# 610265158/Peppa_Pig_Face_Landmark

Hardware: NVIDIA H100
Metric: faces/sec Student@256 batch=256 (higher is better)
Workload: dtype f32

## Files before the change

### peppa_pig_face_landmark_b200/csrc/conv_fpw.cu

```cuda
#include <cuda.h>
#include <cuda_fp16.h>
#include <string.h>

#include "../../include/skps_b200.h"
#include "common.h"
#include "conv_fpw.h"
#include "tc_ptx.h"

namespace skps {

constexpr int FPW_PRODUCER_REGS = 32, FPW_TRANSFORM_REGS = 160, FPW_MMA_REGS = 160;
static_assert(128 * FPW_PRODUCER_REGS + 256 * FPW_TRANSFORM_REGS + 128 * FPW_MMA_REGS <= 65536, "register file split");

__device__ __forceinline__ float2 fpw_ld2(const void* base, int fmt, long long plane, long long i) {
    if (fmt == DT_SPLIT16) {
        const __half* h = (const __half*)base;
        const float2 a = __half22float2(*reinterpret_cast<const __half2*>(h + i));
        const float2 b = __half22float2(*reinterpret_cast<const __half2*>(h + i + plane));
        return make_float2(a.x + b.x, a.y + b.y);
    }
    return *reinterpret_cast<const float2*>((const float*)base + i);
}

template <int N, int KS>
__device__ __forceinline__ void fpw_mma(float* acc, uint64_t a_hi, uint64_t a_lo, uint64_t b_hi, uint64_t b_lo,
                                        uint32_t accumulate) {
    constexpr uint64_t A_HALF = 64 * 128 >> 4;
#pragma unroll
    for (int k = 0; k < KS; ++k) {
        const uint64_t koff = (uint64_t)(k * 32 >> 4);
#pragma unroll
        for (int m = 0; m < 2; ++m)
            wg_mma3<N>(acc + (N / 2) * m, a_hi + m * A_HALF + koff, a_lo + m * A_HALF + koff, b_hi + koff, b_lo + koff,
                       k ? 1u : accumulate);
    }
}

template <int MODE, int N, int ACT, bool OUT_SPLIT>
__global__ void __launch_bounds__(XF_THREADS, 1)
conv_fpw_kernel(const __grid_constant__ CUtensorMap tm0, const __grid_constant__ CUtensorMap tm1_hi,
                const __grid_constant__ CUtensorMap tm1_lo, const __grid_constant__ CUtensorMap tmB_hi,
                const __grid_constant__ CUtensorMap tmB_lo, const __grid_constant__ CUtensorMap tmO_hi,
                const __grid_constant__ CUtensorMap tmO_lo, const __grid_constant__ CUtensorMap tmW,
                const __grid_constant__ FpwK p) {
    extern __shared__ uint8_t smem_raw[];
    __shared__ __align__(8) XfBarriers bar;

    const int warp = threadIdx.x >> 5, lane = threadIdx.x & 31;
    const uint32_t b_plane = (uint32_t)N * 128u, b_slot = 2u * b_plane;
    const XfSmem sm = xf_smem<MODE>(smem_raw, p.a, p.bs, b_slot, p.out_bufs);
    xf_cta_init<MODE>(p.a, bar, sm, smem_raw, &tm0, &tm1_hi, &tmB_hi, &tmB_lo);
    if (warp < 4) {
        asm volatile("setmaxnreg.dec.sync.aligned.u32 %0;" ::"n"(FPW_PRODUCER_REGS));
    if (warp == 0) {
        if (lane == 0) {
            int st = 0, bst = 0;
            uint32_t ph = 0, bph = 0;
            for (int u = blockIdx.x; u < p.units; u += gridDim.x) {
                const int tile = u / p.nsplit, nh = u - tile * p.nsplit;
                const int img = tile / p.a.tiles_per_img, t = tile - img * p.a.tiles_per_img;
                const int oy0 = (t / p.a.tiles_x) * XF_TH, ox0 = (t % p.a.tiles_x) * XF_TW;
                for (int kc = 0; kc < p.a.cchunks; ++kc) {
                    mbar_wait_g(smem_u32(&bar.b_empty[bst]), bph ^ 1u);
                    const uint32_t fb = smem_u32(&bar.b_full[bst]);
                    mbar_expect_tx(fb, b_slot);
                    const uint32_t dst = sm.b_off + (uint32_t)bst * b_slot;
                    tma_load_2d(dst, &tmB_hi, fb, kc * 64, nh * N);
                    tma_load_2d(dst + b_plane, &tmB_lo, fb, kc * 64, nh * N);
                    if (++bst == p.bs) { bst = 0; bph ^= 1u; }
                    xf_load_a<MODE>(p.a, bar, sm, &tm0, &tm1_hi, &tm1_lo, &tmW, kc, img, oy0, ox0, st, ph);
                }
            }
        }
    }
    } else if (warp >= 8) {
        asm volatile("setmaxnreg.inc.sync.aligned.u32 %0;" ::"n"(FPW_TRANSFORM_REGS));
        xf_transform<MODE>(p.a, bar, sm, smem_raw, p.units, [&](int u) { return u / p.nsplit; });
    } else if (warp >= 4) {
        asm volatile("setmaxnreg.inc.sync.aligned.u32 %0;" ::"n"(FPW_MMA_REGS));
        const int q = warp & 3;
        const bool leader = q == 0 && lane == 0;
        int ast = 0, bst = 0;
        uint32_t aph = 0, bph = 0;
        int store_i = 0;
        for (int u = blockIdx.x; u < p.units; u += gridDim.x) {
            const int tile = u / p.nsplit, nh = u - tile * p.nsplit;
            float acc[N];
            int prev_a = 0, prev_b = 0;
            for (int kc = 0; kc < p.a.cchunks; ++kc) {
                mbar_wait_g(smem_u32(&bar.a_full[ast]), aph);
                mbar_wait_g(smem_u32(&bar.b_full[bst]), bph);
                const uint32_t sa = sm.a_off + (uint32_t)ast * XF_A_BYTES, sb = sm.b_off + (uint32_t)bst * b_slot;
                const uint64_t a_hi = make_smem_desc(sa), a_lo = make_smem_desc(sa + XF_A_PLANE);
                const uint64_t b_hi = make_smem_desc(sb), b_lo = make_smem_desc(sb + b_plane);
                const uint32_t accumulate = kc != 0;
                wg_fence_acc(acc);
                switch (p.a.chunk_ksteps[kc]) {
                    case 4: wg_fence(); fpw_mma<N, 4>(acc, a_hi, a_lo, b_hi, b_lo, accumulate); wg_commit(); break;
                    case 3: wg_fence(); fpw_mma<N, 3>(acc, a_hi, a_lo, b_hi, b_lo, accumulate); wg_commit(); break;
                    case 2: wg_fence(); fpw_mma<N, 2>(acc, a_hi, a_lo, b_hi, b_lo, accumulate); wg_commit(); break;
                    default: wg_fence(); fpw_mma<N, 1>(acc, a_hi, a_lo, b_hi, b_lo, accumulate); wg_commit(); break;
                }
                wg_fence_acc(acc);
                wg_wait<1>();
                wg_fence_acc(acc);
                if (kc > 0 && lane == 0) {
                    mbar_arrive(smem_u32(&bar.a_empty[prev_a]));
                    mbar_arrive(smem_u32(&bar.b_empty[prev_b]));
                }
                prev_a = ast; prev_b = bst;
                if (++ast == p.a.as) { ast = 0; aph ^= 1u; }
                if (++bst == p.bs) { bst = 0; bph ^= 1u; }
            }
            wg_wait<0>();
            wg_fence_acc(acc);
            if (lane == 0) {
                mbar_arrive(smem_u32(&bar.a_empty[prev_a]));
                mbar_arrive(smem_u32(&bar.b_empty[prev_b]));
            }
            const int img = tile / p.a.tiles_per_img, t = tile - img * p.a.tiles_per_img;
            const int ty0 = (t / p.a.tiles_x) * XF_TH, tx0 = (t % p.a.tiles_x) * XF_TW;
            const long long pix0 = ((long long)img * p.a.H + ty0) * p.a.W + tx0;
#pragma unroll
            for (int s = 0; s < (N + 31) / 32; ++s) {
                const int co = nh * N + 32 * s;
                if (co >= p.Cout) break;
                const uint32_t sbuf = sm.o_off + (uint32_t)(store_i % p.out_bufs) * XF_OUT_BUF;
                if (leader) {
                    if (p.out_bufs == 2) asm volatile("cp.async.bulk.wait_group.read 1;" ::: "memory");
                    else asm volatile("cp.async.bulk.wait_group.read 0;" ::: "memory");
                }
                ++store_i;
                asm volatile("bar.sync 1, 128;" ::: "memory");
                float bias[8];
#pragma unroll
                for (int i = 0; i < 4; ++i)
#pragma unroll
                    for (int j = 0; j < 2; ++j) {
                        const int c = co + 8 * i + 2 * (lane & 3) + j;
                        bias[2 * i + j] = c < p.Cout ? __ldg(p.bias + c) : 0.f;
                    }
#pragma unroll
                for (int m = 0; m < 2; ++m)
#pragma unroll
                    for (int h = 0; h < 2; ++h) {
                        const int r = 64 * m + 16 * q + (lane >> 2) + 8 * h;
#pragma unroll
                        for (int i = 0; i < 4; ++i) {
                            if (32 * s + 8 * i >= N) continue;
                            const float* a = acc + (N / 2) * m + 4 * (4 * s + i) + 2 * h;
                            float v0 = fmaf(a[0], p.out_scale, bias[2 * i]);
                            float v1 = fmaf(a[1], p.out_scale, bias[2 * i + 1]);
                            if (p.res && co + 8 * i < p.Cout) {
                                const long long pix = pix0 + (r / XF_TW) * p.a.W + r % XF_TW;
                                const float2 rv = fpw_ld2(p.res, p.res_fmt, p.res_plane,
                                                          pix * p.res_ld + p.res_coff + co + 8 * i + 2 * (lane & 3));
                                if (p.res_first) { v0 = act_t<ACT>(v0 + rv.x); v1 = act_t<ACT>(v1 + rv.y); }
                                else { v0 = act_t<ACT>(v0) + rv.x; v1 = act_t<ACT>(v1) + rv.y; }
                            } else {
                                v0 = act_t<ACT>(v0); v1 = act_t<ACT>(v1);
                            }
                            if (OUT_SPLIT) {
                                const __half2 h2 = __floats2half2_rn(v0, v1);
                                const float2 hf = __half22float2(h2);
                                const __half2 l2 = __floats2half2_rn(v0 - hf.x, v1 - hf.y);
                                const uint32_t addr = sbuf + (uint32_t)r * 64u + (uint32_t)((i ^ (r >> 1)) & 3) * 16u +
                                                      (uint32_t)(lane & 3) * 4u;
                                asm volatile("st.shared.b32 [%0], %1;" ::"r"(addr), "r"(*reinterpret_cast<const uint32_t*>(&h2)) : "memory");
                                asm volatile("st.shared.b32 [%0], %1;" ::"r"(addr + 8192u), "r"(*reinterpret_cast<const uint32_t*>(&l2)) : "memory");
                            } else {
                                const uint32_t addr = sbuf + (uint32_t)r * 128u +
                                                      (uint32_t)(((2 * i + ((lane & 3) >> 1)) ^ r) & 7) * 16u +
                                                      (uint32_t)(lane & 1) * 8u;
                                asm volatile("st.shared.v2.f32 [%0], {%1, %2};" ::"r"(addr), "f"(v0), "f"(v1) : "memory");
                            }
                        }
                    }
                asm volatile("fence.proxy.async.shared::cta;" ::: "memory");
                asm volatile("bar.sync 1, 128;" ::: "memory");
                if (leader) {
                    asm volatile("cp.async.bulk.tensor.4d.global.shared::cta.bulk_group [%0, {%2, %3, %4, %5}], [%1];"
                                 ::"l"(&tmO_hi), "r"(sbuf), "r"(co), "r"(tx0), "r"(ty0), "r"(img) : "memory");
                    if (OUT_SPLIT)
                        asm volatile("cp.async.bulk.tensor.4d.global.shared::cta.bulk_group [%0, {%2, %3, %4, %5}], [%1];"
                                     ::"l"(&tmO_lo), "r"(sbuf + 8192u), "r"(co), "r"(tx0), "r"(ty0), "r"(img) : "memory");
                    asm volatile("cp.async.bulk.commit_group;" ::: "memory");
                }
            }
        }
        if (leader) asm volatile("cp.async.bulk.wait_group 0;" ::: "memory");
    }
}

static int fpw_unit_width(int mode, int n_tile) {
    const int n = n_tile <= 64 ? n_tile : 64;
    if (mode == XF_DW) return n == 32 || n == 64 ? n : 0;
    return n == 48 || n == 64 ? n : 0;
}

bool fpw_supported(const XfSetup& s) {
    if (!xf_supported(s)) return false;
    if (s.act != ACT_NONE && s.act != ACT_RELU) return false;
    if (!fpw_unit_width(s.mode, s.n_tile)) return false;
    const TView& o = s.out;
    if (o.fmt != DT_SPLIT16 && o.fmt != DT_F32) return false;
    const size_t oes = o.fmt == DT_SPLIT16 ? 2 : 4;
    if (o.c_stride != 1 || (s.Cout % 8) || ((size_t)o.ld * oes) % 16 || ((size_t)o.c_off * oes) % 16) return false;
    if (((uintptr_t)o.base % 16) || (o.fmt == DT_SPLIT16 && ((size_t)o.plane * 2) % 16)) return false;
    if (o.H % XF_TH || o.W % XF_TW) return false;
    if (s.res.base) {
        if (s.res.c_stride != 1 || (s.res.fmt != DT_SPLIT16 && s.res.fmt != DT_F32)) return false;
        if (s.res.H != o.H || s.res.W != o.W || s.res.C < s.Cout || ((s.res.ld | s.res.c_off) & 1) || (s.res.plane & 1))
            return false;
    }
    XfProducer a;
    a.cchunks = ((s.low.base ? s.low.C : 0) + s.x.C + 63) / 64;
    int bs, out_bufs;
    return xf_rings(a, s.mode, (size_t)fpw_unit_width(s.mode, s.n_tile) * 256, 0, true, bs, out_bufs) != 0;
}

int fpw_prepare(FpwLayer& L, const XfSetup& s) {
    SKPS_CHECK(fpw_supported(s), "conv_fpw: unsupported layer");
    EncodeTiledFn enc = tensor_map_encoder();
    SKPS_CHECK(enc, "cuTensorMapEncodeTiled entry point not available");
    memset(&L.k, 0, sizeof(L.k));
    FpwK& k = L.k;
    L.mode = s.mode;
    L.n = fpw_unit_width(s.mode, s.n_tile);
    L.act = s.act;
    L.out_fmt = s.out.fmt;
    const TView& out = s.out;
    if (xf_producer_prepare(k.a, L.src0, L.src1_hi, L.src1_lo, L.w_eff, s)) return 1;
    k.nsplit = (s.n_tile + L.n - 1) / L.n;
    const int K_pad = k.a.cchunks * 64;
    for (int plane = 0; plane < 2; ++plane) {
        cuuint64_t dims[2] = {(cuuint64_t)K_pad, (cuuint64_t)s.n_tile};
        cuuint64_t strides[1] = {(cuuint64_t)K_pad * 2};
        cuuint32_t box[2] = {64, (cuuint32_t)L.n};
        cuuint32_t estr[2] = {1, 1};
        CUresult r = enc(plane ? &L.b_lo : &L.b_hi, CU_TENSOR_MAP_DATA_TYPE_FLOAT16, 2, (void*)(plane ? s.w_lo : s.w_hi), dims,
                         strides, box, estr, CU_TENSOR_MAP_INTERLEAVE_NONE, CU_TENSOR_MAP_SWIZZLE_128B,
                         CU_TENSOR_MAP_L2_PROMOTION_L2_256B, CU_TENSOR_MAP_FLOAT_OOB_FILL_NONE);
        SKPS_CHECK(r == CUDA_SUCCESS, "conv_fpw: cuTensorMapEncodeTiled(B) failed: %d", (int)r);
    }
    const bool split = out.fmt == DT_SPLIT16;
    const int oes = split ? 2 : 4;
    for (int plane = 0; plane < (split ? 2 : 1); ++plane) {
        cuuint64_t dims[4] = {(cuuint64_t)s.Cout, (cuuint64_t)out.W, (cuuint64_t)out.H, (cuuint64_t)s.max_batch};
        cuuint64_t strides[3] = {(cuuint64_t)out.ld * oes, (cuuint64_t)out.W * out.ld * oes,
                                 (cuuint64_t)out.H * out.W * out.ld * oes};
        cuuint32_t box[4] = {32, XF_TW, XF_TH, 1};
        cuuint32_t estr[4] = {1, 1, 1, 1};
        char* base = (char*)out.base + (size_t)out.c_off * oes + (plane ? (size_t)out.plane * 2 : 0);
        CUresult r = enc(plane ? &L.o_lo : &L.o_hi, split ? CU_TENSOR_MAP_DATA_TYPE_FLOAT16 : CU_TENSOR_MAP_DATA_TYPE_FLOAT32,
                         4, base, dims, strides, box, estr, CU_TENSOR_MAP_INTERLEAVE_NONE,
                         split ? CU_TENSOR_MAP_SWIZZLE_64B : CU_TENSOR_MAP_SWIZZLE_128B, CU_TENSOR_MAP_L2_PROMOTION_NONE,
                         CU_TENSOR_MAP_FLOAT_OOB_FILL_NONE);
        SKPS_CHECK(r == CUDA_SUCCESS, "conv_fpw: cuTensorMapEncodeTiled(out) failed: %d", (int)r);
    }
    if (!split) L.o_lo = L.o_hi;
    const size_t smem = xf_rings(k.a, s.mode, (size_t)L.n * 256, 0, true, k.bs, k.out_bufs);
    SKPS_CHECK(smem, "conv_fpw: layer does not fit shared memory");
    L.smem_bytes = (int)smem + 1024;
    k.Cout = s.Cout; k.out_scale = s.out_scale;
    k.bias = s.bias ? s.bias : zero_bias();
    SKPS_CHECK(k.bias, "conv_fpw: zero-bias allocation failed");
    k.res = s.res.base; k.res_fmt = s.res.fmt; k.res_plane = s.res.plane; k.res_ld = s.res.ld; k.res_coff = s.res.c_off;
    k.res_first = s.res.base ? s.res_first : 0;
    return 0;
}

template <int MODE, int N, int ACT, bool SPLIT>
static int fpw_launch_t(const FpwLayer& L, const FpwK& k, int grid, cudaStream_t stream) {
    static int attr_bytes[MAX_DEVICES] = {};
    if (smem_limit((const void*)conv_fpw_kernel<MODE, N, ACT, SPLIT>, attr_bytes, L.smem_bytes)) return 1;
    conv_fpw_kernel<MODE, N, ACT, SPLIT><<<grid, XF_THREADS, L.smem_bytes, stream>>>(
        L.src0, L.src1_hi, L.src1_lo, L.b_hi, L.b_lo, L.o_hi, L.o_lo, L.w_eff, k);
    SKPS_CUDA(cudaGetLastError());
    return 0;
}

template <int MODE, int N>
static int fpw_launch_n(const FpwLayer& L, const FpwK& k, int grid, cudaStream_t stream) {
    const bool sp = L.out_fmt == DT_SPLIT16;
    switch (L.act) {
        case ACT_NONE: return sp ? fpw_launch_t<MODE, N, ACT_NONE, true>(L, k, grid, stream) : fpw_launch_t<MODE, N, ACT_NONE, false>(L, k, grid, stream);
        case ACT_RELU: return sp ? fpw_launch_t<MODE, N, ACT_RELU, true>(L, k, grid, stream) : fpw_launch_t<MODE, N, ACT_RELU, false>(L, k, grid, stream);
        default: break;
    }
    set_error("conv_fpw: activation %d not instantiated", L.act);
    return 1;
}

Grid fpw_grid(const FpwLayer& L, int batch, int num_sms, FpwK* kp) {
    FpwK k = L.k;
    k.units = batch * k.a.tiles_per_img * k.nsplit;
    if (kp) *kp = k;
    return persistent_grid(k.units, num_sms);
}

int fpw_launch(const FpwLayer& L, int batch, int num_sms, cudaStream_t stream) {
    FpwK k;
    const int grid = fpw_grid(L, batch, num_sms, &k).ctas;
    if (L.mode == XF_DW) {
        switch (L.n) {
            case 32: return fpw_launch_n<XF_DW, 32>(L, k, grid, stream);
            case 64: return fpw_launch_n<XF_DW, 64>(L, k, grid, stream);
            default: break;
        }
    } else {
        switch (L.n) {
            case 48: return fpw_launch_n<XF_SCALE, 48>(L, k, grid, stream);
            case 64: return fpw_launch_n<XF_SCALE, 64>(L, k, grid, stream);
            default: break;
        }
    }
    set_error("conv_fpw: mode %d width %d not instantiated", L.mode, L.n);
    return 1;
}

}
```

### peppa_pig_face_landmark_b200/csrc/conv_fpw.h

```cpp
#pragma once
#include <cuda.h>
#include <cuda_runtime.h>
#include <stdint.h>

#include "xf_producer.h"

namespace skps {

struct FpwK {
    XfProducer a;
    int units;
    int nsplit;
    int bs, out_bufs;
    int Cout;
    float out_scale;
    const float* bias;
    const void* res; int res_fmt; long long res_plane; int res_ld, res_coff; int res_first;
};

struct FpwLayer {
    CUtensorMap src0, src1_hi, src1_lo, b_hi, b_lo, o_hi, o_lo, w_eff;
    FpwK k;
    int mode = 0, n = 0, act = 0, out_fmt = 0;
    int smem_bytes = 0;
};

bool fpw_supported(const XfSetup& s);
int fpw_prepare(FpwLayer& L, const XfSetup& s);
Grid fpw_grid(const FpwLayer& L, int batch, int num_sms, FpwK* k = nullptr);
int fpw_launch(const FpwLayer& L, int batch, int num_sms, cudaStream_t stream);

}
```

### peppa_pig_face_landmark_b200/csrc/xf_producer.h

```cpp
#pragma once
#include <cuda.h>
#include <cuda_fp16.h>
#include <cuda_runtime.h>
#include <stdint.h>

#include "common.h"
#include "tc_ptx.h"

namespace skps {

enum { XF_SCALE = 0, XF_DW = 1 };
enum { XS_UP_F32 = 0, XS_DW_F32 = 1, XS_DW_SPLIT = 2 };
constexpr int XF_MAX_CHUNKS = 16;

constexpr int XF_THREADS = 512;
constexpr int XF_TW = 16, XF_TH = 8;
constexpr int XF_IW = XF_TW + 2, XF_IH = XF_TH + 2;
constexpr int XF_LW = XF_TW / 2 + 2, XF_LH = XF_TH / 2 + 2;
constexpr int XF_RAW_BYTES = XF_IH * XF_IW * 128;
constexpr int XF_UP_BYTES = XF_LH * XF_LW * 128;
constexpr int XF_A_PLANE = 128 * 128;
constexpr int XF_A_BYTES = 2 * XF_A_PLANE;
constexpr int XF_RING = 4;
constexpr int XF_OUT_BUF = 16384;

struct XfSetup {
    int mode;
    int max_batch;
    TView x, low, gate;
    const float* dww;
    const float* weff;
    int dw_act;
    int Cout, act, n_tile, n_tiles;
    float out_scale;
    const void* w_hi; const void* w_lo;
    const float* bias;
    TView out, res;
    int res_first;
};

struct XfProducer {
    int H, W, tiles_x, tiles_per_img;
    int cchunks, Cin;
    int rs, as;
    int dw_act;
    int Hl, Wl;
    int halves;
    int wcx;
    uint8_t sub_mode[2 * XF_MAX_CHUNKS];
    int16_t sub_c[2 * XF_MAX_CHUNKS];
    uint8_t chunk_subs[XF_MAX_CHUNKS];
    uint8_t chunk_ksteps[XF_MAX_CHUNKS];
    const float* dww;
    const float* gate; int gate_ld, gate_coff;
};

bool xf_supported(const XfSetup& s);
int xf_producer_prepare(XfProducer& k, CUtensorMap& src0, CUtensorMap& src1_hi, CUtensorMap& src1_lo, CUtensorMap& w_eff,
                        const XfSetup& s);
size_t xf_rings(XfProducer& k, int mode, size_t b_slot, size_t reserve, bool two_out_bufs, int& bs, int& out_bufs);

struct XfBarriers {
    uint64_t raw_full[XF_RING], raw_empty[XF_RING], a_raw[XF_RING], a_full[XF_RING], a_empty[XF_RING], b_full[XF_RING],
        b_empty[XF_RING];
};

struct XfSmem {
    uint32_t a_off, b_off, o_off, r_off, w_off;
};

template <int MODE>
__device__ __forceinline__ XfSmem xf_smem(const uint8_t* smem_raw, const XfProducer& p, int bs, uint32_t b_slot, int out_bufs) {
    XfSmem s;
    s.a_off = (smem_u32(smem_raw) + 1023u) & ~1023u;
    s.b_off = s.a_off + (uint32_t)p.as * XF_A_BYTES;
    s.o_off = s.b_off + (uint32_t)bs * b_slot;
    s.r_off = s.o_off + (uint32_t)out_bufs * XF_OUT_BUF;
    s.w_off = s.r_off + (MODE == XF_DW ? (uint32_t)p.rs * XF_RAW_BYTES : 0u);
    return s;
}

template <int MODE>
__device__ __forceinline__ void xf_cta_init(const XfProducer& p, XfBarriers& bar, const XfSmem& sm, uint8_t* smem_raw,
                                            const CUtensorMap* tm0, const CUtensorMap* tm1_hi, const CUtensorMap* tmB_hi,
                                            const CUtensorMap* tmB_lo) {
    const int warp = threadIdx.x >> 5, lane = threadIdx.x & 31;
    if (warp == 0 && lane == 0) {
        asm volatile("prefetch.tensormap [%0];" ::"l"(tm0) : "memory");
        asm volatile("prefetch.tensormap [%0];" ::"l"(tm1_hi) : "memory");
        asm volatile("prefetch.tensormap [%0];" ::"l"(tmB_hi) : "memory");
        asm volatile("prefetch.tensormap [%0];" ::"l"(tmB_lo) : "memory");
    }
    if (warp == 1 && lane == 0) {
        for (int s = 0; s < XF_RING; ++s) {
            mbar_init(smem_u32(&bar.raw_full[s]), 1);
            mbar_init(smem_u32(&bar.raw_empty[s]), p.halves ? 4 : 8);
            mbar_init(smem_u32(&bar.a_raw[s]), 1);
            mbar_init(smem_u32(&bar.a_full[s]), 8);
            mbar_init(smem_u32(&bar.a_empty[s]), 4);
            mbar_init(smem_u32(&bar.b_full[s]), 1);
            mbar_init(smem_u32(&bar.b_empty[s]), 4);
        }
        asm volatile("fence.mbarrier_init.release.cluster;" ::: "memory");
    }
    if (MODE == XF_DW) {
        float* dws = reinterpret_cast<float*>(smem_raw + (sm.w_off - smem_u32(smem_raw)));
        for (int i = threadIdx.x; i < 10 * p.cchunks * 64; i += XF_THREADS) dws[i] = __ldg(p.dww + i);
    }
    __syncthreads();
}

template <int MODE>
__device__ __forceinline__ void xf_load_a(const XfProducer& p, XfBarriers& bar, const XfSmem& sm, const CUtensorMap* tm0,
                                          const CUtensorMap* tm1_hi, const CUtensorMap* tm1_lo, const CUtensorMap* tmW,
                                          int kc, int img, int oy0, int ox0, int& st, uint32_t& ph) {
    if (MODE == XF_SCALE) {
        mbar_wait_g(smem_u32(&bar.a_empty[st]), ph ^ 1u);
        const uint32_t fb = smem_u32(&bar.a_raw[st]);
        mbar_expect_tx(fb, XF_A_BYTES);
        const uint32_t dst = sm.a_off + (uint32_t)st * XF_A_BYTES;
        tma_load_4d(dst, tm1_hi, fb, kc * 64, ox0, oy0, img);
        tma_load_4d(dst + XF_A_PLANE, tm1_lo, fb, kc * 64, ox0, oy0, img);
        if (++st == p.as) { st = 0; ph ^= 1u; }
        return;
    }
    const int subs = p.chunk_subs[kc];
    for (int h = 0; h < subs; ++h) {
        const int si = kc * 2 + h, smode = p.sub_mode[si], c = p.sub_c[si];
        mbar_wait_g(smem_u32(&bar.raw_empty[st]), ph ^ 1u);
        const uint32_t fb = smem_u32(&bar.raw_full[st]);
        const uint32_t dst = sm.r_off + (uint32_t)st * XF_RAW_BYTES;
        if (smode == XS_UP_F32) {
            mbar_expect_tx(fb, XF_UP_BYTES + (uint32_t)p.wcx * 3u * 9u * 128u);
            tma_load_4d(dst, tm0, fb, c, (ox0 >> 1) - 1, (oy0 >> 1) - 1, img);
            tma_load_5d(dst + XF_UP_BYTES, tmW, fb, 0, 0, (p.wcx == 4 || ox0 == 0) ? 0 : 1, oy0 == 0 ? 0 : 1, c >> 5);
        } else if (smode == XS_DW_F32) {
            mbar_expect_tx(fb, XF_RAW_BYTES);
            tma_load_4d(dst, tm0, fb, c, ox0 - 1, oy0 - 1, img);
        } else {
            mbar_expect_tx(fb, XF_RAW_BYTES);
            tma_load_4d(dst, tm1_hi, fb, c, ox0 - 1, oy0 - 1, img);
            tma_load_4d(dst + XF_RAW_BYTES / 2, tm1_lo, fb, c, ox0 - 1, oy0 - 1, img);
        }
        if (++st == p.rs) { st = 0; ph ^= 1u; }
    }
}

__device__ __forceinline__ void split_store4(uint32_t addr_hi, const float4 v) {
    const __half2 h01 = __floats2half2_rn(v.x, v.y), h23 = __floats2half2_rn(v.z, v.w);
    const float2 f01 = __half22float2(h01), f23 = __half22float2(h23);
    const __half2 l01 = __floats2half2_rn(v.x - f01.x, v.y - f01.y), l23 = __floats2half2_rn(v.z - f23.x, v.w - f23.y);
    asm volatile("st.shared.v2.b32 [%0], {%1, %2};" ::"r"(addr_hi), "r"(*reinterpret_cast<const uint32_t*>(&h01)),
                 "r"(*reinterpret_cast<const uint32_t*>(&h23)) : "memory");
    asm volatile("st.shared.v2.b32 [%0], {%1, %2};" ::"r"(addr_hi + (uint32_t)XF_A_PLANE),
                 "r"(*reinterpret_cast<const uint32_t*>(&l01)), "r"(*reinterpret_cast<const uint32_t*>(&l23)) : "memory");
}
__device__ __forceinline__ float4 f4_fma(const float4 a, const float4 w, const float4 c) {
    return make_float4(fmaf(a.x, w.x, c.x), fmaf(a.y, w.y, c.y), fmaf(a.z, w.z, c.z), fmaf(a.w, w.w, c.w));
}

template <int ACT>
__device__ __forceinline__ void act16(float4* acc) {
#pragma unroll
    for (int q = 0; q < 4; ++q) {
        acc[q].x = act_t<ACT>(acc[q].x); acc[q].y = act_t<ACT>(acc[q].y);
        acc[q].z = act_t<ACT>(acc[q].z); acc[q].w = act_t<ACT>(acc[q].w);
    }
}

template <int MODE, class TileOf>
__device__ __forceinline__ void xf_transform(const XfProducer& p, XfBarriers& bar, const XfSmem& sm, uint8_t* smem_raw,
                                             int n_work, TileOf tile_of) {
    const int lane = threadIdx.x & 31;
    const int tt = threadIdx.x - 256;
    const int Kpad = p.cchunks * 64;
    int ast = 0, rst = 0;
    uint32_t aph = 0, rph = 0;
    if (MODE == XF_SCALE) {
        const int r0 = tt >> 3, ps = tt & 7, j = ps ^ (r0 & 7);
        for (int u = blockIdx.x; u < n_work; u += gridDim.x) {
            const int img = tile_of(u) / p.tiles_per_img;
            const float* grow = p.gate + (long long)img * p.gate_ld + p.gate_coff;
            for (int kc = 0; kc < p.cchunks; ++kc) {
                const int c = kc * 64 + j * 8;
                float g[8];
                if (c < p.Cin) {
                    const float4 g0 = __ldg(reinterpret_cast<const float4*>(grow + c));
                    const float4 g1 = __ldg(reinterpret_cast<const float4*>(grow + c + 4));
                    g[0] = g0.x; g[1] = g0.y; g[2] = g0.z; g[3] = g0.w; g[4] = g1.x; g[5] = g1.y; g[6] = g1.z; g[7] = g1.w;
                } else {
#pragma unroll
                    for (int e = 0; e < 8; ++e) g[e] = 0.f;
                }
                mbar_wait_g(smem_u32(&bar.a_raw[ast]), aph);
                const uint32_t sa = sm.a_off + (uint32_t)ast * XF_A_BYTES + (uint32_t)ps * 16u;
#pragma unroll
                for (int i = 0; i < 4; ++i) {
                    const uint32_t ad = sa + (uint32_t)(r0 + 32 * i) * 128u;
                    uint32_t hv[4], lv[4];
                    asm volatile("ld.shared.v4.b32 {%0, %1, %2, %3}, [%4];" : "=r"(hv[0]), "=r"(hv[1]), "=r"(hv[2]), "=r"(hv[3]) : "r"(ad) : "memory");
                    asm volatile("ld.shared.v4.b32 {%0, %1, %2, %3}, [%4];" : "=r"(lv[0]), "=r"(lv[1]), "=r"(lv[2]), "=r"(lv[3]) : "r"(ad + (uint32_t)XF_A_PLANE) : "memory");
#pragma unroll
                    for (int e = 0; e < 4; ++e) {
                        const float2 hf = __half22float2(*reinterpret_cast<const __half2*>(&hv[e]));
                        const float2 lf = __half22float2(*reinterpret_cast<const __half2*>(&lv[e]));
                        const float v0 = (hf.x + lf.x) * g[2 * e], v1 = (hf.y + lf.y) * g[2 * e + 1];
                        const __half2 h2 = __floats2half2_rn(v0, v1);
                        const float2 h2f = __half22float2(h2);
                        const __half2 l2 = __floats2half2_rn(v0 - h2f.x, v1 - h2f.y);
                        hv[e] = *reinterpret_cast<const uint32_t*>(&h2);
                        lv[e] = *reinterpret_cast<const uint32_t*>(&l2);
                    }
                    asm volatile("st.shared.v4.b32 [%0], {%1, %2, %3, %4};" ::"r"(ad), "r"(hv[0]), "r"(hv[1]), "r"(hv[2]), "r"(hv[3]) : "memory");
                    asm volatile("st.shared.v4.b32 [%0], {%1, %2, %3, %4};" ::"r"(ad + (uint32_t)XF_A_PLANE), "r"(lv[0]), "r"(lv[1]), "r"(lv[2]), "r"(lv[3]) : "memory");
                }
                asm volatile("fence.proxy.async.shared::cta;" ::: "memory");
                __syncwarp();
                if (lane == 0) mbar_arrive(smem_u32(&bar.a_full[ast]));
                if (++ast == p.as) { ast = 0; aph ^= 1u; }
            }
        }
    } else if (!p.halves) {
        const int cl = tt & 7, pg = tt >> 3, prow = pg >> 2, xs = (pg & 3) * 4;
        const float* dws = reinterpret_cast<const float*>(smem_raw + (sm.w_off - smem_u32(smem_raw)));
        for (int u = blockIdx.x; u < n_work; u += gridDim.x) {
            for (int kc = 0; kc < p.cchunks; ++kc) {
                mbar_wait_g(smem_u32(&bar.a_empty[ast]), aph ^ 1u);
                const uint32_t sa = sm.a_off + (uint32_t)ast * XF_A_BYTES;
                const int subs = p.chunk_subs[kc];
                for (int h = 0; h < subs; ++h) {
                    const int smode = p.sub_mode[kc * 2 + h];
                    const int cw = kc * 64 + h * 32 + cl * 4;
                    const float4 bias4 = *reinterpret_cast<const float4*>(dws + 9 * Kpad + cw);
                    float4 acc[4] = {bias4, bias4, bias4, bias4};
                    mbar_wait_g(smem_u32(&bar.raw_full[rst]), rph);
                    const uint8_t* raw = smem_raw + (sm.r_off + (uint32_t)rst * XF_RAW_BYTES - smem_u32(smem_raw));
                    {
#pragma unroll
                        for (int ky = 0; ky < 3; ++ky) {
                            float4 in[6];
#pragma unroll
                            for (int i = 0; i < 6; ++i) {
                                const int px = (prow + ky) * XF_IW + xs + i;
                                if (smode == XS_DW_F32) {
                                    in[i] = *reinterpret_cast<const float4*>(raw + (px * 32 + cl * 4) * 4);
                                } else {
                                    const uint2 a = *reinterpret_cast<const uint2*>(raw + (px * 32 + cl * 4) * 2);
                                    const uint2 b = *reinterpret_cast<const uint2*>(raw + XF_RAW_BYTES / 2 + (px * 32 + cl * 4) * 2);
                                    const float2 a01 = __half22float2(*reinterpret_cast<const __half2*>(&a.x));
                                    const float2 a23 = __half22float2(*reinterpret_cast<const __half2*>(&a.y));
                                    const float2 b01 = __half22float2(*reinterpret_cast<const __half2*>(&b.x));
                                    const float2 b23 = __half22float2(*reinterpret_cast<const __half2*>(&b.y));
                                    in[i] = make_float4(a01.x + b01.x, a01.y + b01.y, a23.x + b23.x, a23.y + b23.y);
                                }
                            }
#pragma unroll
                            for (int kx = 0; kx < 3; ++kx) {
                                const float4 w = *reinterpret_cast<const float4*>(dws + (ky * 3 + kx) * Kpad + cw);
#pragma unroll
                                for (int q = 0; q < 4; ++q) acc[q] = f4_fma(in[q + kx], w, acc[q]);
// ... 170 lines not shown
```

Measured before the change: 20180.

## Add paired-consumer fused pointwise kernel sharing one A tile across two N halves

After: 20800 (median of 6 runs). 1.03x the previous value.

```diff
diff --git a/peppa_pig_face_landmark_b200/csrc/conv_fpw.cu b/peppa_pig_face_landmark_b200/csrc/conv_fpw.cu
--- a/peppa_pig_face_landmark_b200/csrc/conv_fpw.cu
+++ b/peppa_pig_face_landmark_b200/csrc/conv_fpw.cu
@@ -33,6 +33,152 @@
         for (int m = 0; m < 2; ++m)
             wg_mma3<N>(acc + (N / 2) * m, a_hi + m * A_HALF + koff, a_lo + m * A_HALF + koff, b_hi + koff, b_lo + koff,
                        k ? 1u : accumulate);
+    }
+}
+
+template <int N, int ACT, bool OUT_SPLIT, int PER, bool RES>
+__device__ __forceinline__ void fpw_consumer(const FpwK& p, XfBarriers& bar, const XfSmem& sm, const CUtensorMap* tmO_hi,
+                                             const CUtensorMap* tmO_lo, int wg) {
+    const int warp = threadIdx.x >> 5, lane = threadIdx.x & 31;
+    const uint32_t b_plane = (uint32_t)(PER * N) * 128u, b_slot = 2u * b_plane, b_row = (uint32_t)(wg * N) * 128u;
+    const uint32_t o_base = sm.o_off + (uint32_t)(wg * p.out_bufs) * XF_OUT_BUF, named_bar = 1 + wg;
+    const int items = p.nsplit / PER;
+    const int q = warp & 3;
+    const bool leader = q == 0 && lane == 0;
+    int ast = 0, bst = 0;
+    uint32_t aph = 0, bph = 0;
+    int store_i = 0;
+    for (int u = blockIdx.x; u < p.units; u += gridDim.x) {
+        const int tile = u / items, nh = (u - tile * items) * PER + wg;
+        float acc[N];
+        int prev_a = 0, prev_b = 0;
+        for (int kc = 0; kc < p.a.cchunks; ++kc) {
+            mbar_wait_g(smem_u32(&bar.a_full[ast]), aph);
+            mbar_wait_g(smem_u32(&bar.b_full[bst]), bph);
+            const uint32_t sa = sm.a_off + (uint32_t)ast * XF_A_BYTES, sb = sm.b_off + (uint32_t)bst * b_slot + b_row;
+            const uint64_t a_hi = make_smem_desc(sa), a_lo = make_smem_desc(sa + XF_A_PLANE);
+            const uint64_t b_hi = make_smem_desc(sb), b_lo = make_smem_desc(sb + b_plane);
+            const uint32_t accumulate = kc != 0;
+            wg_fence_acc(acc);
+            switch (p.a.chunk_ksteps[kc]) {
+                case 4: wg_fence(); fpw_mma<N, 4>(acc, a_hi, a_lo, b_hi, b_lo, accumulate); wg_commit(); break;
+                case 3: wg_fence(); fpw_mma<N, 3>(acc, a_hi, a_lo, b_hi, b_lo, accumulate); wg_commit(); break;
+                case 2: wg_fence(); fpw_mma<N, 2>(acc, a_hi, a_lo, b_hi, b_lo, accumulate); wg_commit(); break;
+                default: wg_fence(); fpw_mma<N, 1>(acc, a_hi, a_lo, b_hi, b_lo, accumulate); wg_commit(); break;
+            }
+            wg_fence_acc(acc);
+            wg_wait<1>();
+            wg_fence_acc(acc);
+            if (kc > 0 && lane == 0) {
+                mbar_arrive(smem_u32(&bar.a_empty[prev_a]));
+                mbar_arrive(smem_u32(&bar.b_empty[prev_b]));
+            }
+            prev_a = ast; prev_b = bst;
+            if (++ast == p.a.as) { ast = 0; aph ^= 1u; }
+            if (++bst == p.bs) { bst = 0; bph ^= 1u; }
+        }
+        wg_wait<0>();
+        wg_fence_acc(acc);
+        if (lane == 0) {
+            mbar_arrive(smem_u32(&bar.a_empty[prev_a]));
+            mbar_arrive(smem_u32(&bar.b_empty[prev_b]));
+        }
+        const int img = tile / p.a.tiles_per_img, t = tile - img * p.a.tiles_per_img;
+        const int ty0 = (t / p.a.tiles_x) * XF_TH, tx0 = (t % p.a.tiles_x) * XF_TW;
+        const long long pix0 = ((long long)img * p.a.H + ty0) * p.a.W + tx0;
+#pragma unroll
+        for (int s = 0; s < (N + 31) / 32; ++s) {
+            const int co = nh * N + 32 * s;
+            if (co >= p.Cout) break;
+            const uint32_t sbuf = o_base + (uint32_t)(store_i % p.out_bufs) * XF_OUT_BUF;
+            if (leader) {
+                if (p.out_bufs == 2) asm volatile("cp.async.bulk.wait_group.read 1;" ::: "memory");
+                else asm volatile("cp.async.bulk.wait_group.read 0;" ::: "memory");
+            }
+            ++store_i;
+            asm volatile("bar.sync %0, 128;" ::"r"(named_bar) : "memory");
+            float bias[8];
+#pragma unroll
+            for (int i = 0; i < 4; ++i)
+#pragma unroll
+                for (int j = 0; j < 2; ++j) {
+                    const int c = co + 8 * i + 2 * (lane & 3) + j;
+                    bias[2 * i + j] = c < p.Cout ? __ldg(p.bias + c) : 0.f;
+                }
+#pragma unroll
+            for (int m = 0; m < 2; ++m)
+#pragma unroll
+                for (int h = 0; h < 2; ++h) {
+                    const int r = 64 * m + 16 * q + (lane >> 2) + 8 * h;
+#pragma unroll
+                    for (int i = 0; i < 4; ++i) {
+                        if (32 * s + 8 * i >= N) continue;
+                        const float* a = acc + (N / 2) * m + 4 * (4 * s + i) + 2 * h;
+                        float v0 = fmaf(a[0], p.out_scale, bias[2 * i]);
+                        float v1 = fmaf(a[1], p.out_scale, bias[2 * i + 1]);
+                        if (RES && p.res && co + 8 * i < p.Cout) {
+                            const long long pix = pix0 + (r / XF_TW) * p.a.W + r % XF_TW;
+                            const float2 rv = fpw_ld2(p.res, p.res_fmt, p.res_plane,
+                                                      pix * p.res_ld + p.res_coff + co + 8 * i + 2 * (lane & 3));
+                            if (p.res_first) { v0 = act_t<ACT>(v0 + rv.x); v1 = act_t<ACT>(v1 + rv.y); }
+                            else { v0 = act_t<ACT>(v0) + rv.x; v1 = act_t<ACT>(v1) + rv.y; }
+                        } else {
+                            v0 = act_t<ACT>(v0); v1 = act_t<ACT>(v1);
+                        }
+                        if (OUT_SPLIT) {
+                            const __half2 h2 = __floats2half2_rn(v0, v1);
+                            const float2 hf = __half22float2(h2);
+                            const __half2 l2 = __floats2half2_rn(v0 - hf.x, v1 - hf.y);
+                            const uint32_t addr = sbuf + (uint32_t)r * 64u + (uint32_t)((i ^ (r >> 1)) & 3) * 16u +
+                                                  (uint32_t)(lane & 3) * 4u;
+                            asm volatile("st.shared.b32 [%0], %1;" ::"r"(addr), "r"(*reinterpret_cast<const uint32_t*>(&h2)) : "memory");
+                            asm volatile("st.shared.b32 [%0], %1;" ::"r"(addr + 8192u), "r"(*reinterpret_cast<const uint32_t*>(&l2)) : "memory");
+                        } else {
+                            const uint32_t addr = sbuf + (uint32_t)r * 128u +
+                                                  (uint32_t)(((2 * i + ((lane & 3) >> 1)) ^ r) & 7) * 16u +
+                                                  (uint32_t)(lane & 1) * 8u;
+                            asm volatile("st.shared.v2.f32 [%0], {%1, %2};" ::"r"(addr), "f"(v0), "f"(v1) : "memory");
+                        }
+                    }
+                }
+            asm volatile("fence.proxy.async.shared::cta;" ::: "memory");
+            asm volatile("bar.sync %0, 128;" ::"r"(named_bar) : "memory");
+            if (leader) {
+                asm volatile("cp.async.bulk.tensor.4d.global.shared::cta.bulk_group [%0, {%2, %3, %4, %5}], [%1];"
+                             ::"l"(tmO_hi), "r"(sbuf), "r"(co), "r"(tx0), "r"(ty0), "r"(img) : "memory");
+                if (OUT_SPLIT)
+                    asm volatile("cp.async.bulk.tensor.4d.global.shared::cta.bulk_group [%0, {%2, %3, %4, %5}], [%1];"
+                                 ::"l"(tmO_lo), "r"(sbuf + 8192u), "r"(co), "r"(tx0), "r"(ty0), "r"(img) : "memory");
+                asm volatile("cp.async.bulk.commit_group;" ::: "memory");
+            }
+        }
+    }
+    if (leader) asm volatile("cp.async.bulk.wait_group 0;" ::: "memory");
+}
+
+template <int MODE, int N, int PER>
+__device__ __forceinline__ void fpw_producer(const FpwK& p, XfBarriers& bar, const XfSmem& sm, const CUtensorMap* tm0,
+                                             const CUtensorMap* tm1_hi, const CUtensorMap* tm1_lo,
+                                             const CUtensorMap* tmB_hi, const CUtensorMap* tmB_lo,
+                                             const CUtensorMap* tmW) {
+    const uint32_t b_plane = (uint32_t)(PER * N) * 128u, b_slot = 2u * b_plane;
+    const int items = p.nsplit / PER;
+    int st = 0, bst = 0;
+    uint32_t ph = 0, bph = 0;
+    for (int u = blockIdx.x; u < p.units; u += gridDim.x) {
+        const int tile = u / items, n0 = (u - tile * items) * PER * N;
+        const int img = tile / p.a.tiles_per_img, t = tile - img * p.a.tiles_per_img;
+        const int oy0 = (t / p.a.tiles_x) * XF_TH, ox0 = (t % p.a.tiles_x) * XF_TW;
+        for (int kc = 0; kc < p.a.cchunks; ++kc) {
+            mbar_wait_g(smem_u32(&bar.b_empty[bst]), bph ^ 1u);
+            const uint32_t fb = smem_u32(&bar.b_full[bst]);
+            mbar_expect_tx(fb, b_slot);
+            const uint32_t dst = sm.b_off + (uint32_t)bst * b_slot;
+            tma_load_2d(dst, tmB_hi, fb, kc * 64, n0);
+            tma_load_2d(dst + b_plane, tmB_lo, fb, kc * 64, n0);
+            if (++bst == p.bs) { bst = 0; bph ^= 1u; }
+            xf_load_a<MODE>(p.a, bar, sm, tm0, tm1_hi, tm1_lo, tmW, kc, img, oy0, ox0, st, ph);
+        }
     }
 }
 
@@ -47,148 +193,48 @@
     __shared__ __align__(8) XfBarriers bar;
 
     const int warp = threadIdx.x >> 5, lane = threadIdx.x & 31;
-    const uint32_t b_plane = (uint32_t)N * 128u, b_slot = 2u * b_plane;
-    const XfSmem sm = xf_smem<MODE>(smem_raw, p.a, p.bs, b_slot, p.out_bufs);
+    const XfSmem sm = xf_smem<MODE>(smem_raw, p.a, p.bs, 2u * N * 128u, p.out_bufs);
     xf_cta_init<MODE>(p.a, bar, sm, smem_raw, &tm0, &tm1_hi, &tmB_hi, &tmB_lo);
     if (warp < 4) {
         asm volatile("setmaxnreg.dec.sync.aligned.u32 %0;" ::"n"(FPW_PRODUCER_REGS));
-    if (warp == 0) {
-        if (lane == 0) {
-            int st = 0, bst = 0;
-            uint32_t ph = 0, bph = 0;
-            for (int u = blockIdx.x; u < p.units; u += gridDim.x) {
-                const int tile = u / p.nsplit, nh = u - tile * p.nsplit;
-                const int img = tile / p.a.tiles_per_img, t = tile - img * p.a.tiles_per_img;
-                const int oy0 = (t / p.a.tiles_x) * XF_TH, ox0 = (t % p.a.tiles_x) * XF_TW;
-                for (int kc = 0; kc < p.a.cchunks; ++kc) {
-                    mbar_wait_g(smem_u32(&bar.b_empty[bst]), bph ^ 1u);
-                    const uint32_t fb = smem_u32(&bar.b_full[bst]);
-                    mbar_expect_tx(fb, b_slot);
-                    const uint32_t dst = sm.b_off + (uint32_t)bst * b_slot;
-                    tma_load_2d(dst, &tmB_hi, fb, kc * 64, nh * N);
-                    tma_load_2d(dst + b_plane, &tmB_lo, fb, kc * 64, nh * N);
-                    if (++bst == p.bs) { bst = 0; bph ^= 1u; }
-                    xf_load_a<MODE>(p.a, bar, sm, &tm0, &tm1_hi, &tm1_lo, &tmW, kc, img, oy0, ox0, st, ph);
-                }
-            }
-        }
-    }
+        if (warp == 0 && lane == 0) fpw_producer<MODE, N, 1>(p, bar, sm, &tm0, &tm1_hi, &tm1_lo, &tmB_hi, &tmB_lo, &tmW);
     } else if (warp >= 8) {
         asm volatile("setmaxnreg.inc.sync.aligned.u32 %0;" ::"n"(FPW_TRANSFORM_REGS));
         xf_transform<MODE>(p.a, bar, sm, smem_raw, p.units, [&](int u) { return u / p.nsplit; });
-    } else if (warp >= 4) {
+    } else {
         asm volatile("setmaxnreg.inc.sync.aligned.u32 %0;" ::"n"(FPW_MMA_REGS));
-        const int q = warp & 3;
-        const bool leader = q == 0 && lane == 0;
-        int ast = 0, bst = 0;
-        uint32_t aph = 0, bph = 0;
-        int store_i = 0;
-        for (int u = blockIdx.x; u < p.units; u += gridDim.x) {
-            const int tile = u / p.nsplit, nh = u - tile * p.nsplit;
-            float acc[N];
-            int prev_a = 0, prev_b = 0;
-            for (int kc = 0; kc < p.a.cchunks; ++kc) {
-                mbar_wait_g(smem_u32(&bar.a_full[ast]), aph);
-                mbar_wait_g(smem_u32(&bar.b_full[bst]), bph);
-                const uint32_t sa = sm.a_off + (uint32_t)ast * XF_A_BYTES, sb = sm.b_off + (uint32_t)bst * b_slot;
-                const uint64_t a_hi = make_smem_desc(sa), a_lo = make_smem_desc(sa + XF_A_PLANE);
-                const uint64_t b_hi = make_smem_desc(sb), b_lo = make_smem_desc(sb + b_plane);
-                const uint32_t accumulate = kc != 0;
-                wg_fence_acc(acc);
-                switch (p.a.chunk_ksteps[kc]) {
-                    case 4: wg_fence(); fpw_mma<N, 4>(acc, a_hi, a_lo, b_hi, b_lo, accumulate); wg_commit(); break;
-                    case 3: wg_fence(); fpw_mma<N, 3>(acc, a_hi, a_lo, b_hi, b_lo, accumulate); wg_commit(); break;
-                    case 2: wg_fence(); fpw_mma<N, 2>(acc, a_hi, a_lo, b_hi, b_lo, accumulate); wg_commit(); break;
-                    default: wg_fence(); fpw_mma<N, 1>(acc, a_hi, a_lo, b_hi, b_lo, accumulate); wg_commit(); break;
-                }
-                wg_fence_acc(acc);
-                wg_wait<1>();
-                wg_fence_acc(acc);
-                if (kc > 0 && lane == 0) {
-                    mbar_arrive(smem_u32(&bar.a_empty[prev_a]));
-                    mbar_arrive(smem_u32(&bar.b_empty[prev_b]));
-                }
-                prev_a = ast; prev_b = bst;
-                if (++ast == p.a.as) { ast = 0; aph ^= 1u; }
-                if (++bst == p.bs) { bst = 0; bph ^= 1u; }
-            }
-            wg_wait<0>();
-            wg_fence_acc(acc);
-            if (lane == 0) {
-                mbar_arrive(smem_u32(&bar.a_empty[prev_a]));
-                mbar_arrive(smem_u32(&bar.b_empty[prev_b]));
-            }
-            const int img = tile / p.a.tiles_per_img, t = tile - img * p.a.tiles_per_img;
-            const int ty0 = (t / p.a.tiles_x) * XF_TH, tx0 = (t % p.a.tiles_x) * XF_TW;
-            const long long pix0 = ((long long)img * p.a.H + ty0) * p.a.W + tx0;
-#pragma unroll
-            for (int s = 0; s < (N + 31) / 32; ++s) {
-                const int co = nh * N + 32 * s;
-                if (co >= p.Cout) break;
-                const uint32_t sbuf = sm.o_off + (uint32_t)(store_i % p.out_bufs) * XF_OUT_BUF;
-                if (leader) {
-                    if (p.out_bufs == 2) asm volatile("cp.async.bulk.wait_group.read 1;" ::: "memory");
-                    else asm volatile("cp.async.bulk.wait_group.read 0;" ::: "memory");
-                }
-                ++store_i;
-                asm volatile("bar.sync 1, 128;" ::: "memory");
-                float bias[8];
-#pragma unroll
-                for (int i = 0; i < 4; ++i)
-#pragma unroll
-                    for (int j = 0; j < 2; ++j) {
-                        const int c = co + 8 * i + 2 * (lane & 3) + j;
-                        bias[2 * i + j] = c < p.Cout ? __ldg(p.bias + c) : 0.f;
-                    }
-#pragma unroll
-                for (int m = 0; m < 2; ++m)
-#pragma unroll
-                    for (int h = 0; h < 2; ++h) {
-                        const int r = 64 * m + 16 * q + (lane >> 2) + 8 * h;
-#pragma unroll
-                        for (int i = 0; i < 4; ++i) {
-                            if (32 * s + 8 * i >= N) continue;
-                            const float* a = acc + (N / 2) * m + 4 * (4 * s + i) + 2 * h;
-                            float v0 = fmaf(a[0], p.out_scale, bias[2 * i]);
-                            float v1 = fmaf(a[1], p.out_scale, bias[2 * i + 1]);
-                            if (p.res && co + 8 * i < p.Cout) {
-                                const long long pix = pix0 + (r / XF_TW) * p.a.W + r % XF_TW;
-                                const float2 rv = fpw_ld2(p.res, p.res_fmt, p.res_plane,
-                                                          pix * p.res_ld + p.res_coff + co + 8 * i + 2 * (lane & 3));
-                                if (p.res_first) { v0 = act_t<ACT>(v0 + rv.x); v1 = act_t<ACT>(v1 + rv.y); }
-                                else { v0 = act_t<ACT>(v0) + rv.x; v1 = act_t<ACT>(v1) + rv.y; }
-                            } else {
-                                v0 = act_t<ACT>(v0); v1 = act_t<ACT>(v1);
-                            }
-                            if (OUT_SPLIT) {
-                                const __half2 h2 = __floats2half2_rn(v0, v1);
-                                const float2 hf = __half22float2(h2);
-                                const __half2 l2 = __floats2half2_rn(v0 - hf.x, v1 - hf.y);
-                                const uint32_t addr = sbuf + (uint32_t)r * 64u + (uint32_t)((i ^ (r >> 1)) & 3) * 16u +
-                                                      (uint32_t)(lane & 3) * 4u;
-                                asm volatile("st.shared.b32 [%0], %1;" ::"r"(addr), "r"(*reinterpret_cast<const uint32_t*>(&h2)) : "memory");
-                                asm volatile("st.shared.b32 [%0], %1;" ::"r"(addr + 8192u), "r"(*reinterpret_cast<const uint32_t*>(&l2)) : "memory");
-                            } else {
-                                const uint32_t addr = sbuf + (uint32_t)r * 128u +
-                                                      (uint32_t)(((2 * i + ((lane & 3) >> 1)) ^ r) & 7) * 16u +
-                                                      (uint32_t)(lane & 1) * 8u;
-                                asm volatile("st.shared.v2.f32 [%0], {%1, %2};" ::"r"(addr), "f"(v0), "f"(v1) : "memory");
-                            }
-                        }
-                    }
-                asm volatile("fence.proxy.async.shared::cta;" ::: "memory");
-                asm volatile("bar.sync 1, 128;" ::: "memory");
-                if (leader) {
-                    asm volatile("cp.async.bulk.tensor.4d.global.shared::cta.bulk_group [%0, {%2, %3, %4, %5}], [%1];"
-                                 ::"l"(&tmO_hi), "r"(sbuf), "r"(co), "r"(tx0), "r"(ty0), "r"(img) : "memory");
-                    if (OUT_SPLIT)
-                        asm volatile("cp.async.bulk.tensor.4d.global.shared::cta.bulk_group [%0, {%2, %3, %4, %5}], [%1];"
-                                     ::"l"(&tmO_lo), "r"(sbuf + 8192u), "r"(co), "r"(tx0), "r"(ty0), "r"(img) : "memory");
-                    asm volatile("cp.async.bulk.commit_group;" ::: "memory");
-                }
-            }
-        }
-        if (leader) asm volatile("cp.async.bulk.wait_group 0;" ::: "memory");
+        fpw_consumer<N, ACT, OUT_SPLIT, 1, true>(p, bar, sm, &tmO_hi, &tmO_lo, 0);
+    }
+}
+
+constexpr int FPW_PAIR_THREADS = 640;
+constexpr int FPW_PAIR_PRODUCER_REGS = 24, FPW_PAIR_TRANSFORM_REGS = 120, FPW_PAIR_MMA_REGS = 104;
+static_assert(128 * FPW_PAIR_PRODUCER_REGS + 256 * FPW_PAIR_TRANSFORM_REGS + 256 * FPW_PAIR_MMA_REGS <= FPW_PAIR_THREADS * 96,
+              "register file split");
+
+template <int ACT, bool OUT_SPLIT>
+__global__ void __launch_bounds__(FPW_PAIR_THREADS, 1)
+conv_fpw_pair(const __grid_constant__ CUtensorMap tm0, const __grid_constant__ CUtensorMap tm1_hi,
+              const __grid_constant__ CUtensorMap tm1_lo, const __grid_constant__ CUtensorMap tmB_hi,
+              const __grid_constant__ CUtensorMap tmB_lo, const __grid_constant__ CUtensorMap tmO_hi,
+              const __grid_constant__ CUtensorMap tmO_lo, const __grid_constant__ CUtensorMap tmW,
+              const __grid_constant__ FpwK p) {
+    constexpr int N = 64;
+    extern __shared__ uint8_t smem_raw[];
+    __shared__ __align__(8) XfBarriers bar;
+
+    const int warp = threadIdx.x >> 5, lane = threadIdx.x & 31;
+    const XfSmem sm = xf_smem<XF_DW>(smem_raw, p.a, p.bs, 4u * N * 128u, 2 * p.out_bufs);
+    xf_cta_init<XF_DW>(p.a, bar, sm, smem_raw, &tm0, &tm1_hi, &tmB_hi, &tmB_lo, 8, FPW_PAIR_THREADS);
+    if (warp < 4) {
+        asm volatile("setmaxnreg.dec.sync.aligned.u32 %0;" ::"n"(FPW_PAIR_PRODUCER_REGS));
+        if (warp == 0 && lane == 0) fpw_producer<XF_DW, N, 2>(p, bar, sm, &tm0, &tm1_hi, &tm1_lo, &tmB_hi, &tmB_lo, &tmW);
+    } else if (warp >= 8 && warp < 16) {
+        asm volatile("setmaxnreg.inc.sync.aligned.u32 %0;" ::"n"(FPW_PAIR_TRANSFORM_REGS));
+        xf_transform<XF_DW>(p.a, bar, sm, smem_raw, p.units, [&](int u) { return u / (p.nsplit / 2); });
+    } else {
+        asm volatile("setmaxnreg.inc.sync.aligned.u32 %0;" ::"n"(FPW_PAIR_MMA_REGS));
+        fpw_consumer<N, ACT, OUT_SPLIT, 2, false>(p, bar, sm, &tmO_hi, &tmO_lo, warp < 8 ? 0 : 1);
     }
 }
 
@@ -196,6 +242,17 @@
     const int n = n_tile <= 64 ? n_tile : 64;
     if (mode == XF_DW) return n == 32 || n == 64 ? n : 0;
     return n == 48 || n == 64 ? n : 0;
+}
+
+static bool fpw_pair(const XfSetup& s) {
+    const int n = fpw_unit_width(s.mode, s.n_tile);
+    return s.mode == XF_DW && n == 64 && (s.n_tile + n - 1) / n % 2 == 0 && !s.res.base;
+}
+
+static size_t fpw_rings(XfProducer& a, const XfSetup& s, int& bs, int& out_bufs) {
+    const size_t n = (size_t)fpw_unit_width(s.mode, s.n_tile);
+    if (fpw_pair(s)) return xf_rings(a, s.mode, 2 * n * 256, XF_OUT_BUF, false, bs, out_bufs) + XF_OUT_BUF;
+    return xf_rings(a, s.mode, n * 256, 0, true, bs, out_bufs);
 }
 
 bool fpw_supported(const XfSetup& s) {
@@ -216,7 +273,7 @@
     XfProducer a;
     a.cchunks = ((s.low.base ? s.low.C : 0) + s.x.C + 63) / 64;
     int bs, out_bufs;
-    return xf_rings(a, s.mode, (size_t)fpw_unit_width(s.mode, s.n_tile) * 256, 0, true, bs, out_bufs) != 0;
+    return fpw_rings(a, s, bs, out_bufs) != 0;
 }
 
 int fpw_prepare(FpwLayer& L, const XfSetup& s) {
@@ -227,6 +284,7 @@
     FpwK& k = L.k;
     L.mode = s.mode;
     L.n = fpw_unit_width(s.mode, s.n_tile);
+    L.pair = fpw_pair(s);
     L.act = s.act;
     L.out_fmt = s.out.fmt;
     const TView& out = s.out;
@@ -236,7 +294,7 @@
     for (int plane = 0; plane < 2; ++plane) {
         cuuint64_t dims[2] = {(cuuint64_t)K_pad, (cuuint64_t)s.n_tile};
         cuuint64_t strides[1] = {(cuuint64_t)K_pad * 2};
-        cuuint32_t box[2] = {64, (cuuint32_t)L.n};
+        cuuint32_t box[2] = {64, (cuuint32_t)(L.pair ? 2 * L.n : L.n)};
         cuuint32_t estr[2] = {1, 1};
         CUresult r = enc(plane ? &L.b_lo : &L.b_hi, CU_TENSOR_MAP_DATA_TYPE_FLOAT16, 2, (void*)(plane ? s.w_lo : s.w_hi), dims,
                          strides, box, estr, CU_TENSOR_MAP_INTERLEAVE_NONE, CU_TENSOR_MAP_SWIZZLE_128B,
@@ -259,7 +317,7 @@
         SKPS_CHECK(r == CUDA_SUCCESS, "conv_fpw: cuTensorMapEncodeTiled(out) failed: %d", (int)r);
     }
     if (!split) L.o_lo = L.o_hi;
-    const size_t smem = xf_rings(k.a, s.mode, (size_t)L.n * 256, 0, true, k.bs, k.out_bufs);
+    const size_t smem = fpw_rings(k.a, s, k.bs, k.out_bufs);
     SKPS_CHECK(smem, "conv_fpw: layer does not fit shared memory");
     L.smem_bytes = (int)smem + 1024;
     k.Cout = s.Cout; k.out_scale = s.out_scale;
@@ -280,6 +338,27 @@
     return 0;
 }
 
+template <int ACT, bool SPLIT>
+static int fpw_launch_pair_t(const FpwLayer& L, const FpwK& k, int grid, cudaStream_t stream) {
+    static int attr_bytes[MAX_DEVICES] = {};
+    if (smem_limit((const void*)conv_fpw_pair<ACT, SPLIT>, attr_bytes, L.smem_bytes)) return 1;
+    conv_fpw_pair<ACT, SPLIT><<<grid, FPW_PAIR_THREADS, L.smem_bytes, stream>>>(
+        L.src0, L.src1_hi, L.src1_lo, L.b_hi, L.b_lo, L.o_hi, L.o_lo, L.w_eff, k);
+    SKPS_CUDA(cudaGetLastError());
+    return 0;
+}
+
+static int fpw_launch_pair(const FpwLayer& L, const FpwK& k, int grid, cudaStream_t stream) {
+    const bool sp = L.out_fmt == DT_SPLIT16;
+    switch (L.act) {
+        case ACT_NONE: return sp ? fpw_launch_pair_t<ACT_NONE, true>(L, k, grid, stream) : fpw_launch_pair_t<ACT_NONE, false>(L, k, grid, stream);
+        case ACT_RELU: return sp ? fpw_launch_pair_t<ACT_RELU, true>(L, k, grid, stream) : fpw_launch_pair_t<ACT_RELU, false>(L, k, grid, stream);
+        default: break;
+    }
+    set_error("conv_fpw: activation %d not instantiated", L.act);
+    return 1;
+}
+
 template <int MODE, int N>
 static int fpw_launch_n(const FpwLayer& L, const FpwK& k, int grid, cudaStream_t stream) {
     const bool sp = L.out_fmt == DT_SPLIT16;
@@ -294,7 +373,7 @@
 
 Grid fpw_grid(const FpwLayer& L, int batch, int num_sms, FpwK* kp) {
     FpwK k = L.k;
-    k.units = batch * k.a.tiles_per_img * k.nsplit;
+    k.units = batch * k.a.tiles_per_img * (L.pair ? k.nsplit / 2 : k.nsplit);
     if (kp) *kp = k;
     return persistent_grid(k.units, num_sms);
 }
@@ -302,6 +381,7 @@
 int fpw_launch(const FpwLayer& L, int batch, int num_sms, cudaStream_t stream) {
     FpwK k;
     const int grid = fpw_grid(L, batch, num_sms, &k).ctas;
+    if (L.pair) return fpw_launch_pair(L, k, grid, stream);
     if (L.mode == XF_DW) {
         switch (L.n) {
             case 32: return fpw_launch_n<XF_DW, 32>(L, k, grid, stream);
diff --git a/peppa_pig_face_landmark_b200/csrc/conv_fpw.h b/peppa_pig_face_landmark_b200/csrc/conv_fpw.h
--- a/peppa_pig_face_landmark_b200/csrc/conv_fpw.h
+++ b/peppa_pig_face_landmark_b200/csrc/conv_fpw.h
@@ -22,6 +22,7 @@
     CUtensorMap src0, src1_hi, src1_lo, b_hi, b_lo, o_hi, o_lo, w_eff;
     FpwK k;
     int mode = 0, n = 0, act = 0, out_fmt = 0;
+    bool pair = false;
     int smem_bytes = 0;
 };
 
diff --git a/peppa_pig_face_landmark_b200/csrc/xf_producer.h b/peppa_pig_face_landmark_b200/csrc/xf_producer.h
--- a/peppa_pig_face_landmark_b200/csrc/xf_producer.h
+++ b/peppa_pig_face_landmark_b200/csrc/xf_producer.h
@@ -83,7 +83,7 @@
 template <int MODE>
 __device__ __forceinline__ void xf_cta_init(const XfProducer& p, XfBarriers& bar, const XfSmem& sm, uint8_t* smem_raw,
                                             const CUtensorMap* tm0, const CUtensorMap* tm1_hi, const CUtensorMap* tmB_hi,
-                                            const CUtensorMap* tmB_lo) {
+                                            const CUtensorMap* tmB_lo, int mma_warps = 4, int nthreads = XF_THREADS) {
     const int warp = threadIdx.x >> 5, lane = threadIdx.x & 31;
     if (warp == 0 && lane == 0) {
         asm volatile("prefetch.tensormap [%0];" ::"l"(tm0) : "memory");
@@ -97,15 +97,15 @@
             mbar_init(smem_u32(&bar.raw_empty[s]), p.halves ? 4 : 8);
             mbar_init(smem_u32(&bar.a_raw[s]), 1);
             mbar_init(smem_u32(&bar.a_full[s]), 8);
-            mbar_init(smem_u32(&bar.a_empty[s]), 4);
+            mbar_init(smem_u32(&bar.a_empty[s]), mma_warps);
             mbar_init(smem_u32(&bar.b_full[s]), 1);
-            mbar_init(smem_u32(&bar.b_empty[s]), 4);
+            mbar_init(smem_u32(&bar.b_empty[s]), mma_warps);
         }
         asm volatile("fence.mbarrier_init.release.cluster;" ::: "memory");
     }
     if (MODE == XF_DW) {
         float* dws = reinterpret_cast<float*>(smem_raw + (sm.w_off - smem_u32(smem_raw)));
-        for (int i = threadIdx.x; i < 10 * p.cchunks * 64; i += XF_THREADS) dws[i] = __ldg(p.dww + i);
+        for (int i = threadIdx.x; i < 10 * p.cchunks * 64; i += nthreads) dws[i] = __ldg(p.dww + i);
     }
     __syncthreads();
 }
```
